# nico-bohlinger/RL-X

Hardware: AMD Instinct MI355X
Metric: env-steps/sec (whole node) PPO 4096 envs at 1/2/4/8 MI355X (higher is better)
Workload: dtype f32

## Files before the change

### rl-x_amd/csrc/gemm_bx.hip

```cpp
#include "gemm_bx.h"
#ifndef RLX_WS_MIN_WAVES
#define RLX_WS_MIN_WAVES 2
#endif
#include "mlp.h"

namespace rlx {

__global__ __launch_bounds__(256) void k_bx_wfrag(BxJobs jobs) {
  int ji = 0;
#pragma unroll
  for (int q = 1; q < BX_MAX_JOBS; ++q)
    if (q < jobs.n && (int)blockIdx.x >= jobs.job[q].first_block) ji = q;
  const BxJob& jb = jobs.job[ji];
  const int idx = ((int)blockIdx.x - jb.first_block) * 256 + threadIdx.x;
  if (idx >= jb.KB * jb.NT * 64) return;
  const int lane = idx & 63, blk = idx >> 6, nt = blk % jb.NT, kb = blk / jb.NT;
  const int j = nt * 32 + (lane & 31), k0 = kb * 16 + 8 * (lane >> 5);
  float v[8];
#pragma unroll
  for (int e = 0; e < 8; ++e) {
    const int k = k0 + e;
    v[e] = (k < jb.K && j < jb.N) ? (jb.trans ? jb.W[(int64_t)j * jb.ldw + k] : jb.W[(int64_t)k * jb.ldw + j]) : 0.f;
  }
  u32x4 pl[X_NP];
// ... 128 lines not shown
#pragma unroll
        for (int j = 0; j < 2; ++j)
#pragma unroll
          for (int r = 0; r < 16; ++r) h[j][r] = hsb[(i * 32 + (r & 3) + 8 * (r >> 2)) * ldc + j * 32];
#pragma unroll
        for (int j = 0; j < 2; ++j)
#pragma unroll
          for (int r = 0; r < 16; ++r)
            cb[(i * 32 + (r & 3) + 8 * (r >> 2)) * ldc + j * 32] = acc[i][j][r] * so * act_grad_t<ACT>(h[j][r]);
      }
    } else {
#pragma unroll
      for (int i = 0; i < MI; ++i)
#pragma unroll
        for (int j = 0; j < 2; ++j)
#pragma unroll
          for (int r = 0; r < 16; ++r) cb[(i * 32 + (r & 3) + 8 * (r >> 2)) * ldc + j * 32] = acc[i][j][r] * so;
    }
    return;
  }
#pragma unroll
  for (int j = 0; j < 2; ++j) {
    const int col = n0 + acc_col(wn, j, lane);
    if (col >= N) continue;
#pragma unroll
    for (int i = 0; i < MI; ++i)
#pragma unroll
      for (int r = 0; r < 16; ++r) {
        const int64_t row = m0 + wm * 32 * MI + i * 32 + (r & 3) + 8 * (r >> 2) + 4 * (lane >> 5);
        if (row < M) {
          const int64_t o = row * ldc + col;
          float v = acc[i][j][r] * so;
          if (MODE == 0) v = act_fwd_t<ACT>(v + bv[j]);
          else if (APPLY) v *= act_grad_t<ACT>((Hsrc ? Hsrc : C)[o]);
          C[o] = v;
        }
      }
  }
}

constexpr int XW_THREADS = 512;
struct DwArgs {
  const float* Hp;
  const float* dZ;
  float* partW;
  float* partB;
  const float *Hp1, *dZ1;
  float *partW1, *partB1;
  int64_t M, Mc;
  int Kd, ldh, N, ntk, ntn;
  BxDwRecompute rc;
};
template <bool TWIN, bool REC = false>
__global__ __launch_bounds__(XW_THREADS, 2) void k_gemm_dw_bx(DwArgs a, DwArgs b, int nb0, float sg, float so) {
  extern __shared__ __attribute__((aligned(16))) char lds[];
  int bid = blockIdx.x, nblk = nb0;
  if (bid >= nb0) {
    a = b;
    bid -= nb0;
    nblk = gridDim.x - nb0;
  }
  const float* __restrict__ Hp = a.Hp;
  const float* __restrict__ dZ = a.dZ;
  float* __restrict__ partW = a.partW;
  float* __restrict__ partB = a.partB;
  if (TWIN && blockIdx.y) {
    Hp = a.Hp1;
    dZ = a.dZ1;
    partW = a.partW1;
    partB = a.partB1;
  }
  const int64_t M = a.M, Mc = a.Mc;
  const int Kd = a.Kd, ldh = a.ldh, N = a.N, ntk = a.ntk, ntn = a.ntn;
  const int ntiles = ntk * ntn;
  const int lb = xcd_remap(bid, nblk);
  const int s = lb / ntiles, tile = lb % ntiles;
  const int k0d = (tile / ntn) * G_BM;
  const int n0 = (tile % ntn) * G_BN;
  const int64_t mbeg = (int64_t)s * Mc;
  int64_t mend = mbeg + Mc;
  if (mend > M) mend = M;
  const int t = threadIdx.x, lane = t & 63, wv = t >> 6;
  const int nk = (int)((mend - mbeg + X_BK - 1) / X_BK);
  const bool interior = k0d + G_BM <= Kd && n0 + G_BN <= N;
  float colsum[4] = {0.f, 0.f, 0.f, 0.f};
  const int pt = t & 255, op = pt >> 7, tt = pt & 127, cg = tt & 31, mg = tt >> 5;
  const bool rec = REC && a.rc.X != nullptr;
  if (REC && wv >= 4 && rec && op == 0) {
    const BxDwRecompute& R = a.rc;
    const int wh = wv - 4, li = lane & 31, lh = lane >> 5;
    const int O = R.O;
    const int64_t pdelta = (TWIN && blockIdx.y) ? R.pdelta1 : 0;
    const float* __restrict__ stats = (TWIN && blockIdx.y) ? R.stats1 : R.stats;
    const u32x4* __restrict__ W1x = reinterpret_cast<const u32x4*>((TWIN && blockIdx.y) ? R.W1x1 : R.W1x);
    const float xs = R.xmax ? x_scale_from_max(*R.xmax, X_ASCALE) : X_ASCALE;
    const float xinv = 1.0f / xs;
    u32x4 w1f[2][2][X_NP];
    float bias[2], gam[2], bet[2];
#pragma unroll
    for (int j = 0; j < 2; ++j) {
      const int ctg = (k0d >> 5) + 2 * wh + j;
#pragma unroll
      for (int kb = 0; kb < 2; ++kb)
#pragma unroll
        for (int p = 0; p < X_NP; ++p) w1f[kb][j][p] = W1x[((int64_t)(kb * R.NT1 + ctg) * X_NP + p) * 64 + lane];
      const int col = k0d + 32 * (2 * wh + j) + li;
      bias[j] = R.b1[pdelta + col];
      gam[j] = R.g[pdelta + col];
      bet[j] = R.be[pdelta + col];
    }
    char* xa = lds + 4 * X_OPER + wh * (X_NP * 2048 + 256);
    float* st_l = reinterpret_cast<float*>(xa + X_NP * 2048);
    for (int i = lane; i < X_NP * 2048 / 16; i += 64) reinterpret_cast<u32x4*>(xa)[i] = u32x4{0u, 0u, 0u, 0u};
    constexpr int XC = 9;
    int xr_[XC], xk_[XC];
#pragma unroll
    for (int c = 0; c < XC; ++c) {
      const int e = lane + 64 * c;
      xr_[c] = e / O;
      xk_[c] = e - xr_[c] * O;
    }
    float xv[XC], smean = 0.f, srstd = 0.f;
    auto xload = [&](int kt) {
      const int64_t m0 = mbeg + (int64_t)kt * X_BK;
      const float* xb = R.X + m0 * O;
      const int nvalid = (int)((mend - m0 < X_BK ? mend - m0 : X_BK)) * O;
#pragma unroll
      for (int c = 0; c < XC; ++c) {
        const int e = lane + 64 * c;
        xv[c] = e < nvalid ? xb[e] : 0.f;
      }
      const bool rv = lane < 32 && m0 + lane < mend;
      smean = rv ? stats[m0 + lane] : 0.f;
      srstd = rv ? stats[M + m0 + lane] : 0.f;
    };
    auto produce = [&](int buf) {
#pragma unroll
      for (int c = 0; c < XC; ++c) {
        if (lane + 64 * c < 32 * O) {
          uint32_t p0, p1;
          bx_split2(xv[c] * xs, 0.f, p0, p1);
          char* da = xa + bx_off(xr_[c], xk_[c] >> 3) + (xk_[c] & 7) * 2;
          *reinterpret_cast<uint16_t*>(da) = (uint16_t)p0;
          *reinterpret_cast<uint16_t*>(da + 2048) = (uint16_t)p1;
        }
      }
      if (lane < 32) { st_l[lane] = smean; st_l[32 + lane] = srstd; }
      f32x16 z[2];
#pragma unroll
      for (int j = 0; j < 2; ++j)
#pragma unroll
        for (int r = 0; r < 16; ++r) z[j][r] = bias[j] * (xs * X_WSCALE);
      const int nks = O > 16 ? 2 : 1;
      for (int kb = 0; kb < nks; ++kb) {
        u32x4 xf[X_NP];
#pragma unroll
        for (int p = 0; p < X_NP; ++p) xf[p] = *reinterpret_cast<const u32x4*>(xa + p * 2048 + bx_off(li, 2 * kb + lh));
#pragma unroll
        for (int j = 0; j < 2; ++j) {
          z[j] = __builtin_amdgcn_mfma_f32_32x32x16_f16(__builtin_bit_cast(f16x8, xf[0]), __builtin_bit_cast(f16x8, w1f[kb][j][1]), z[j], 0, 0, 0);
          z[j] = __builtin_amdgcn_mfma_f32_32x32x16_f16(__builtin_bit_cast(f16x8, xf[1]), __builtin_bit_cast(f16x8, w1f[kb][j][0]), z[j], 0, 0, 0);
          z[j] = __builtin_amdgcn_mfma_f32_32x32x16_f16(__builtin_bit_cast(f16x8, xf[0]), __builtin_bit_cast(f16x8, w1f[kb][j][0]), z[j], 0, 0, 0);
        }
      }
      const float zs = xinv * X_WINV;
      char* dst = lds + buf * 2 * X_OPER;
#pragma unroll
      for (int s8 = 0; s8 < 2; ++s8) {
        float4 mv[2], rv[2];
#pragma unroll
        for (int h2 = 0; h2 < 2; ++h2) {
          mv[h2] = *reinterpret_cast<const float4*>(st_l + 16 * s8 + 8 * h2 + 4 * lh);
          rv[h2] = *reinterpret_cast<const float4*>(st_l + 32 + 16 * s8 + 8 * h2 + 4 * lh);
        }
#pragma unroll
        for (int j = 0; j < 2; ++j) {
          float v[8];
#pragma unroll
          for (int e = 0; e < 8; ++e) {
            const float mean = e < 4 ? (&mv[0].x)[e & 3] : (&mv[1].x)[e & 3];
            const float rs = e < 4 ? (&rv[0].x)[e & 3] : (&rv[1].x)[e & 3];
            const float y = fmaf((z[j][8 * s8 + e] * zs - mean) * rs, gam[j], bet[j]);
            v[e] = y > 0.f ? y : __expf(fminf(y, 0.f)) - 1.0f;
          }
          bx_stage_k8<true>(dst, 32 * (2 * wh + j) + li, 2 * s8 + lh, v, X_ASCALE);
        }
      }
    };
    xload(0);
    produce(0);
    if (nk > 1) xload(1);
    __syncthreads();
    for (int kt = 0; kt < nk; ++kt) {
      if (kt + 1 < nk) {
        produce((kt + 1) & 1);
        if (kt + 2 < nk) xload(kt + 2);
      }
      __syncthreads();
    }
    if (k0d == 0 && partB) {
      const float* red = reinterpret_cast<const float*>(lds);
      __syncthreads();
      if (pt < 128 && n0 + pt < N) partB[(int64_t)s * N + n0 + pt] = (red[pt] + red[128 + pt]) + (red[256 + pt] + red[384 + pt]);
    }
    return;
  }
  if (wv >= 4) {
    const float* __restrict__ src = op ? dZ : Hp;
    const int ld = op ? N : ldh, c0 = (op ? n0 : k0d) + cg * 4, ncols = op ? N : Kd;
    const bool plain = interior && (mend - mbeg) % X_BK == 0;
    float4 rra[8];
    const int rbase = rec ? 16 * (mg >> 1) + 4 * (mg & 1) : mg * 8;
    const float* sp = src + (mbeg + rbase) * ld + c0;
    auto load_plain = [&](int kt, float4 (&rr)[8]) {
      const int64_t m0 = (int64_t)kt * X_BK;
#pragma unroll
      for (int e = 0; e < 8; ++e) rr[e] = *reinterpret_cast<const float4*>(sp + (m0 + (rec ? (e & 3) + 8 * (e >> 2) : e)) * ld);
    };
    auto load_edge = [&](int kt, float4 (&rr)[8]) {
      const int64_t m0 = (int64_t)kt * X_BK;
#pragma unroll
      for (int e = 0; e < 8; ++e) rr[e] = ld4(src, mbeg + m0 + rbase + (rec ? (e & 3) + 8 * (e >> 2) : e), c0, mend, ncols, ld);
    };
    const float sc = op ? sg : X_ASCALE;
    auto stage = [&](int buf, const float4 (&rr)[8]) {
      char* dst = lds + buf * 2 * X_OPER + op * X_OPER;
      float v[8];
#pragma unroll
      for (int e = 0; e < 8; ++e) v[e] = rr[e].x;
      bx_stage_k8<true>(dst, cg * 4 + 0, mg, v, sc);
      if (op) {
#pragma unroll
        for (int e = 0; e < 8; ++e) colsum[0] += v[e];
      }
#pragma unroll
      for (int e = 0; e < 8; ++e) v[e] = rr[e].y;
      bx_stage_k8<true>(dst, cg * 4 + 1, mg, v, sc);
      if (op) {
#pragma unroll
        for (int e = 0; e < 8; ++e) colsum[1] += v[e];
      }
#pragma unroll
      for (int e = 0; e < 8; ++e) v[e] = rr[e].z;
      bx_stage_k8<true>(dst, cg * 4 + 2, mg, v, sc);
      if (op) {
#pragma unroll
        for (int e = 0; e < 8; ++e) colsum[2] += v[e];
      }
#pragma unroll
      for (int e = 0; e < 8; ++e) v[e] = rr[e].w;
      bx_stage_k8<true>(dst, cg * 4 + 3, mg, v, sc);
      if (op) {
// ... 383 lines not shown
    RLX_HIP_TRY(hipFuncSetAttribute(reinterpret_cast<const void*>(k_gemm_dw_bx<true>), hipFuncAttributeMaxDynamicSharedMemorySize,
                                    4 * X_OPER + 16384));
    RLX_HIP_TRY(hipFuncSetAttribute(reinterpret_cast<const void*>(k_gemm_dw_bx<false, true>), hipFuncAttributeMaxDynamicSharedMemorySize,
                                    4 * X_OPER + 16384));
    RLX_HIP_TRY(hipFuncSetAttribute(reinterpret_cast<const void*>(k_gemm_dw_bx<true, true>), hipFuncAttributeMaxDynamicSharedMemorySize,
                                    4 * X_OPER + 16384));
    attr_set.mark();  
  }
  return RLX_OK;
}

static DwArgs dw_args(const float* Hp, const float* dZ, float* pW, float* pB, int64_t M, int Kd, int ldh, int N, int64_t Mc, int ntk,
                      int ntn, const Twin* tw) {
  DwArgs a;
  a.Hp = Hp; a.dZ = dZ; a.partW = pW; a.partB = pB;
  a.Hp1 = tw ? static_cast<const float*>(tw->p[0]) : nullptr;
  a.dZ1 = tw ? static_cast<const float*>(tw->p[1]) : nullptr;
  a.partW1 = tw ? const_cast<float*>(static_cast<const float*>(tw->p[2])) : nullptr;
  a.partB1 = tw ? const_cast<float*>(static_cast<const float*>(tw->p[3])) : nullptr;
  a.M = M; a.Mc = Mc; a.Kd = Kd; a.ldh = ldh; a.N = N; a.ntk = ntk; a.ntn = ntn;
  a.rc = BxDwRecompute{};
  return a;
}
constexpr size_t DW_REC_LDS = 2 * (X_NP * 2048 + 256);

int bx_launch_dw(rlx_ctx* ctx, const float* Hp, const float* dZ, float* pW, float* pB, int64_t M, int Kd, int ldh, int N,
                 int64_t Mc, int S, int ntk, int ntn, hipStream_t st, const Twin* tw) {
  int rc = dw_attr();
  if (rc) return rc;
  const float gs = ctx->bx_gscale;
  ProfScope prof(ctx, PK_GEMM_DW, (tw ? 4.0 : 2.0) * (double)M * Kd * N, st, (tw ? 2.0 : 1.0) * gemm_bytes(Kd, N, M), Kd, N, (int)M, 1);
  const DwArgs a = dw_args(Hp, dZ, pW, pB, M, Kd, ldh, N, Mc, ntk, ntn, tw);
  const int nb = S * ntk * ntn;
  if (tw) {
    RLX_PLAUNCH(k_gemm_dw_bx<true>, dim3(nb, 2), dim3(XW_THREADS), 4 * X_OPER, st, a, a, nb, gs, X_AINV / gs);
  } else {
    RLX_PLAUNCH(k_gemm_dw_bx<false>, dim3(nb), dim3(XW_THREADS), 4 * X_OPER, st, a, a, nb, gs, X_AINV / gs);
  }
  RLX_LAUNCH_CHECK();
  return RLX_OK;
}

int bx_launch_dw2(rlx_ctx* ctx, const BxDwJob& j0, const BxDwJob& j1, int64_t M, hipStream_t st, const Twin* tw0, const Twin* tw1) {
  int rc = dw_attr();
  if (rc) return rc;
  RLX_REQUIRE((tw0 == nullptr) == (tw1 == nullptr), RLX_EINVAL, "bx_launch_dw2: both jobs or neither must have a twin");
  const float gs = ctx->bx_gscale;
  const double nets = tw0 ? 2.0 : 1.0;
  ProfScope prof(ctx, PK_GEMM_DW, nets * 2.0 * (double)M * ((double)j0.Kd * j0.N + (double)j1.Kd * j1.N), st,
                 nets * (gemm_bytes(j0.Kd, j0.N, M) + gemm_bytes(j1.Kd, j1.N, M)), j0.Kd + j1.Kd, j0.N + j1.N, (int)M, 1);
  DwArgs a = dw_args(j0.Hp, j0.dZ, j0.pW, j0.pB, M, j0.Kd, j0.ldh, j0.N, j0.Mc, j0.ntk, j0.ntn, tw0);
  const DwArgs b = dw_args(j1.Hp, j1.dZ, j1.pW, j1.pB, M, j1.Kd, j1.ldh, j1.N, j1.Mc, j1.ntk, j1.ntn, tw1);
  if (j0.rc) {
    RLX_REQUIRE(j0.rc->X && j0.rc->W1x && j0.rc->stats && j0.Kd == 512 && j0.rc->O <= 32 && (!tw0 || (j0.rc->W1x1 && j0.rc->stats1)),
                RLX_EINVAL, "bx_launch_dw2: incomplete recompute description");
    a.rc = *j0.rc;
  }
  const int nb0 = j0.S * j0.ntk * j0.ntn, nb1 = j1.S * j1.ntk * j1.ntn;
  const size_t lds = 4 * X_OPER + (j0.rc ? DW_REC_LDS : 0);
  if (j0.rc) {
    if (tw0) { RLX_PLAUNCH((k_gemm_dw_bx<true, true>), dim3(nb0 + nb1, 2), dim3(XW_THREADS), lds, st, a, b, nb0, gs, X_AINV / gs); }
    else { RLX_PLAUNCH((k_gemm_dw_bx<false, true>), dim3(nb0 + nb1), dim3(XW_THREADS), lds, st, a, b, nb0, gs, X_AINV / gs); }
  } else if (tw0) {
    RLX_PLAUNCH(k_gemm_dw_bx<true>, dim3(nb0 + nb1, 2), dim3(XW_THREADS), lds, st, a, b, nb0, gs, X_AINV / gs);
  } else {
    RLX_PLAUNCH(k_gemm_dw_bx<false>, dim3(nb0 + nb1), dim3(XW_THREADS), lds, st, a, b, nb0, gs, X_AINV / gs);
  }
  RLX_LAUNCH_CHECK();
  return RLX_OK;
}

}
```

### rl-x_amd/csrc/mlp.h

```cpp
#pragma once
#include "gemm.h"

namespace rlx {

constexpr int REDUCE_MAX_SEGS = 48;
constexpr int REDUCE_MAX_BLOCKS = 4096;

struct ReduceSeg {
  const float* src;
  float* dst;
  int64_t len;
  int64_t stride;
  int S;
  int nblocks;
  float scale;
  float bias;
  int in_norm;
  int vec;
};
struct ReduceTable {
  int n;
  ReduceSeg seg[REDUCE_MAX_SEGS];
};

// ... 82 lines not shown
int launch_fwd3h(rlx_ctx* ctx, const rlx_mlp_desc& d, const MlpLayout& L, const float* params, const void* const* wx, const float* x, int ldx,
                 float* z1, float* h1, float* h2, float* h3, float* out, int64_t M, hipStream_t st, const Fwd3hTwin* tw = nullptr);
struct Dxa2hTwin {
  const float* params;
  const void* w2t;
  const float *h1, *h2, *dq;
  float* da;
};
bool dxa2h_supported(const rlx_ctx* ctx, const rlx_mlp_desc& d, int64_t M, int nc);
int launch_dxa2h(rlx_ctx* ctx, const rlx_mlp_desc& d, const MlpLayout& L, const float* params, const void* w2t, const float* h1,
                 const float* h2, const float* dq, float* da, int c0, int nc, int ld_da, int64_t M, hipStream_t st,
                 const Dxa2hTwin* tw = nullptr);
bool dw_merge_ok(const rlx_ctx* ctx, const rlx_mlp_desc& d, const MlpLayout& L, int64_t M);
size_t l1fused_partial_floats(const rlx_mlp_desc& d, int grid);
int l1fused_grid(int64_t M, int num_cus);
struct L1FusedTwin {
  const float* params;
  const float* dZ2;
  float* arena;
  float* grads;
  const void *w2x, *w1x;
  ReduceTable* tab;
};
bool l1fused_bx_images(const rlx_ctx* ctx, const MlpLayout& L, const float* params, const void** w2x, const void** w1x);
int launch_l1fused(rlx_ctx* ctx, const rlx_mlp_desc& d, const MlpLayout& L, const float* params, const float* x,
                   const float* dZ2, float* arena, int grid, float* grads, int64_t M, ReduceTable* tab, hipStream_t st,
                   const L1FusedTwin* tw = nullptr);

int bx_prepare_mlp(rlx_ctx* ctx, const rlx_mlp_desc& d, const MlpLayout& L, const float* params, bool with_bwd, hipStream_t st);
void bx_release(rlx_ctx* ctx);
struct BxNetSpec {
  const rlx_mlp_desc* d;
  const float* params;
  bool with_bwd;
  bool first_layer;
};
int bx_prepare_nets(rlx_ctx* ctx, const BxNetSpec* nets, int n_nets, hipStream_t st, ScratchSlot slot = SL_WFRAG, bool launch = true);
struct BxMat {
  const float* W;
  int K, N;
  bool fwd, trans;
};
int bx_prepare_mats(rlx_ctx* ctx, const BxMat* mats, int n, hipStream_t st);
void bx_release_all(rlx_ctx* ctx);
const void* bx_lookup(const rlx_ctx* ctx, const float* W, int trans, int K, int N);
bool bx_twin_usable(const rlx_ctx* ctx, int64_t M, int N);
int bx_launch_fwd(rlx_ctx* ctx, const float* A, const void* img, const float* bias, float* C, int64_t M, int N, int K, int act,
                  hipStream_t st, int lda, const int32_t* m_dev, const Twin* tw = nullptr);
int bx_launch_dx(rlx_ctx* ctx, const float* dZ, const void* img, float* HD, int64_t M, int N, int Kd, int ldo, int act, int apply,
                 hipStream_t st, const Twin* tw = nullptr, const float* hsrc = nullptr);
bool bx_dw_usable(const rlx_ctx* ctx, int64_t M, int Kd, int ldh, int N);
int bx_launch_dw(rlx_ctx* ctx, const float* Hp, const float* dZ, float* pW, float* pB, int64_t M, int Kd, int ldh, int N,
                 int64_t Mc, int S, int ntk, int ntn, hipStream_t st, const Twin* tw = nullptr);
struct BxDwRecompute {
  const float* X = nullptr;
  const void* W1x = nullptr;
  const float* b1 = nullptr;
  const float* g = nullptr;
  const float* be = nullptr;
  const float* stats = nullptr;
  const uint32_t* xmax = nullptr;
  const void* W1x1 = nullptr;
  const float* stats1 = nullptr;
  int64_t pdelta1 = 0;
  int O = 0, NT1 = 16;
};
struct BxDwJob {
  const float* Hp;
  const float* dZ;
  float *pW, *pB;
  int Kd, ldh, N;
  int64_t Mc;
  int S, ntk, ntn;
  const BxDwRecompute* rc = nullptr;
};
int bx_launch_dw2(rlx_ctx* ctx, const BxDwJob& j0, const BxDwJob& j1, int64_t M, hipStream_t st, const Twin* tw0 = nullptr,
                  const Twin* tw1 = nullptr);


struct BxEmitLayer {
  int64_t w_off;
  int in, out;
  void* nn;
  void* tt;
  int nt_nn, nt_tt;
};
struct BxEmit {
  int n;
  BxEmitLayer l[3];
};
BxEmit bx_emit_table(const rlx_ctx* ctx, const rlx_mlp_desc& d, const float* params);
int launch_clip_adam(float* params, const float* grads, float* m, float* v, int64_t n, const float* sumsq_partials,
                     int n_partials, int64_t step, float lr, float max_norm, float b1, float b2, float eps,
                     float* norm_out, hipStream_t st, const float* sched_dev = nullptr, const BxEmit* emit = nullptr,
                     float* polyak_target = nullptr, float tau = 0.f,
                     float weight_decay = 0.f,
                     int clip_mode = 0);
int launch_clip_adam2(float* p0, const float* g0, float* m0, float* v0, int64_t n0, const float* part0, int np0, float* norm0,
                      const BxEmit* e0, float* p1, const float* g1, float* m1, float* v1, int64_t n1, const float* part1, int np1,
                      float* norm1, const BxEmit* e1, int64_t step, float lr, float max_norm, float b1, float b2, float eps,
                      hipStream_t st, const float* sched_dev = nullptr);
int launch_sumsq_partials2(const float* g0, int64_t n0, float* part0, int* np0, const float* g1, int64_t n1, float* part1, int* np1,
                           hipStream_t st);
int clip_adam_step(rlx_ctx* ctx, float* params, const float* grads, float* m, float* v, int64_t n_params, int64_t step, float lr,
                   float max_grad_norm, float b1, float b2, float eps, float* grad_norm_out, hipStream_t st, const BxEmit* emit);
void adam_schedule_entry(float* out3, int64_t step, float lr, float b1, float b2);
// ... 4 lines not shown
```

### rl-x_amd/csrc/ppo.hip

```cpp
#include "ppo_internal.h"
#include "gemm_bx.h"
#include "dist.h"

namespace rlx {

constexpr float LOG_2PI = 1.8378770664093453f;
constexpr float HALF_LOG_2PIE = 1.4189385332046727f;
constexpr int HEAD_ROWS = 64;

__global__ __launch_bounds__(256) void k_gather(const float* __restrict__ states, const float* __restrict__ actions,
                                                const float* __restrict__ logp, const float* __restrict__ returns,
                                                const float* __restrict__ adv, const int32_t* __restrict__ idx,
                                                float* __restrict__ mb_x, float* __restrict__ mb_a,
                                                float* __restrict__ aux, const int32_t* __restrict__ valid_rows,
                                                int64_t mb, int O, int A, const float* __restrict__ cstates,
                                                float* __restrict__ mb_xc, int Oc) {
  const int64_t nv = valid_rows ? (int64_t)*valid_rows : mb;
  const int64_t nx = mb * O, na = mb * A, nxc = cstates ? mb * Oc : 0;
  const int64_t total = nx + na + mb + nxc;
  for (int64_t e = (int64_t)blockIdx.x * 256 + threadIdx.x; e < total; e += (int64_t)gridDim.x * 256) {
    if (e >= nx + na + mb) {
      const int64_t f = e - nx - na - mb;
      const int64_t r = f / Oc;
      const int d = (int)(f - r * Oc);
// ... 1153 lines not shown
    if (REFILL) {                                                                                                     \
      _Pragma("unroll") for (int j = 0; j < JW; ++j) _Pragma("unroll") for (int p = 0; p < X_NP; ++p)                  \
          bc[u][j][p] = wt[(int64_t)((QU) + PFC) * wstep + (j * X_NP + p) * 64];                                       \
    }                                                                                                                 \
    __builtin_amdgcn_sched_barrier(0);                                                                                \
  }
    static_assert(NBC % PFC == 0 && NBC >= PFC, "phase C: whole groups of PFC blocks");
#pragma unroll 1
    for (int q = 0; q < NBC - PFC; q += PFC) {
#pragma unroll
      for (int u = 0; u < PFC; ++u) T32C_BLOCK(q + u, true)
    }
#pragma unroll
    for (int u = 0; u < PFC; ++u) T32C_BLOCK(NBC - PFC + u, false)
#undef T32C_BLOCK
    const float so2 = X_WINV / gs;
#pragma unroll
    for (int j = 0; j < JW; ++j) {
      const int col = (w * JW + j) * 32 + li;
      float* cb = n.dZ2 + (m0 + 4 * lh) * N2 + col;
      const char* hb = H2P + (4 * lh) * HROW + col * 2;
#pragma unroll
      for (int rr = 0; rr < 16; ++rr) {
        const int rho = (rr & 3) + 8 * (rr >> 2);
        const _Float16 hi = *reinterpret_cast<const _Float16*>(hb + rho * HROW);
        const _Float16 lo = *reinterpret_cast<const _Float16*>(hb + rho * HROW + HPL);
        const float h2 = ((float)hi + (float)lo) * X_AINV;
        cb[(int64_t)rho * N2] = acc[j][rr] * so2 * act_grad_t<ACT>(h2);
      }
    }
  }
}

template <int ACT, int N2>
__global__ __launch_bounds__(256, 2) void k_tail32_bx(TailNet p, TailNet c, const float* __restrict__ mb_a,
                                                      const float* __restrict__ aux, const double* __restrict__ stats,
                                                      float* __restrict__ metrics, int64_t M, float inv_mb, float clip,
                                                      float ent_coef, float critic_coef, const int32_t* __restrict__ valid_rows,
                                                      float gs, int both, int which) {
  extern __shared__ __attribute__((aligned(16))) char tl32_smem[];
  const bool critic = both ? blockIdx.y != 0 : which != 0;
  if (!critic)
    tail32_body<true, ACT, N2>(p, tl32_smem, mb_a, aux, stats, metrics, M, inv_mb, clip, ent_coef, critic_coef, valid_rows, gs);
  else
    tail32_body<false, ACT, N2>(c, tl32_smem, mb_a, aux, stats, metrics, M, inv_mb, clip, ent_coef, critic_coef, valid_rows, gs);
}

static inline int tail_rows(const rlx_ctx* ctx, int N2, int act, int64_t mb) {
  const bool can32 = N2 == 256 && act == RLX_ACT_ELU && mb % T32_ROWS == 0;
  const bool want32 = ctx->ppo_tail == 2 || (ctx->ppo_tail < 0 && (mb <= 8192 || mb > 16384));
  return (can32 && want32) ? T32_ROWS : HEAD_ROWS;
}

static bool tail_shape_ok(const rlx_ctx* ctx, const rlx_mlp_desc& d, int64_t mb, const rlx_ppo_hparams& hp) {
  return ctx->ppo_tail && ctx->gemm_bx && !hp.discrete_actions && d.n_hidden == 3 && d.hidden[2] == TL_K3 && d.hidden[1] % G_BN == 0 &&
         d.hidden[1] <= 512 && d.out_dim <= 8 && mb >= 4096 && mb % HEAD_ROWS == 0;
}

static int launch_tail(rlx_ctx* ctx, const TailNet* p, const TailNet* c, const MbScratch& s, float* metrics, int64_t mb, int N2,
                       int mb_global, const rlx_ppo_hparams& hp, int act, hipStream_t st) {
  const TailNet dummy{};
  const TailNet& tp = p ? *p : dummy;
  const TailNet& tc = c ? *c : dummy;
  const int both = (p && c) ? 1 : 0, which = p ? 0 : 1;
  const float gs = bx_grad_scale(mb_global);
  const float inv_mb = 1.0f / (float)mb_global;
  const size_t lds = 2 * X_OPER + (size_t)HEAD_ROWS * TL_TS * sizeof(float);
  const double nets = both ? 2.0 : 1.0;
  ProfScope prof(s.valid_rows ? nullptr : ctx, PK_TAIL, nets * 4.0 * (double)mb * N2 * TL_K3, st,
                 nets * 4.0 * ((double)mb * (2 * N2 + TL_K3) + 2.0 * N2 * TL_K3), mb, TL_K3, N2, 1);
  if (tail_rows(ctx, N2, act, mb) == T32_ROWS) {
    constexpr int HPL = T32_ROWS * (2 * 256 + 16), DPL = T32_ROWS * (2 * TL_K3 + 16);
    constexpr int TREG = (T32_ROWS * TL_TS * 4 > 2 * DPL) ? T32_ROWS * TL_TS * 4 : 2 * DPL;
    const size_t lds32 = 2 * HPL + TREG + ((size_t)TL_K3 * 8 + 2 * T32_ROWS * 8 + 16 + 2 * TL_K3 * 8) * sizeof(float);
    static AttrOnce attr32;
    if (!attr32.done()) {
      RLX_HIP_TRY(hipFuncSetAttribute(reinterpret_cast<const void*>(k_tail32_bx<RLX_ACT_ELU, 256>),
                                      hipFuncAttributeMaxDynamicSharedMemorySize, 160 * 1024));
      attr32.mark();
    }
    RLX_PLAUNCH((k_tail32_bx<RLX_ACT_ELU, 256>), dim3((unsigned)(mb / T32_ROWS), both ? 2 : 1), dim3(256), lds32, st, tp, tc, s.mb_a,
                s.aux, s.stats, metrics, mb, inv_mb, hp.clip_range, hp.entropy_coef, hp.critic_coef, s.valid_rows, gs, both, which);
    RLX_LAUNCH_CHECK();
    return RLX_OK;
  }
#define RLX_TAIL_LAUNCH(ACTV)                                                                                        \
  {                                                                                                                  \
    static AttrOnce attr_set;                                                                                          \
    if (!attr_set.done()) {                                                                                                 \
      RLX_HIP_TRY(hipFuncSetAttribute(reinterpret_cast<const void*>(k_tail_bx<ACTV>),                                \
                                      hipFuncAttributeMaxDynamicSharedMemorySize, 160 * 1024));                      \
      attr_set.mark();                                                                                                 \
    }                                                                                                                \
    RLX_PLAUNCH((k_tail_bx<ACTV>), dim3((unsigned)(mb / HEAD_ROWS), both ? 2 : 1), dim3(256), lds, st, tp, tc, s.mb_a, s.aux,   \
                s.stats, metrics, mb, N2, inv_mb, hp.clip_range, hp.entropy_coef, hp.critic_coef, s.valid_rows, gs, both,      \
                which);                                                                                              \
  }
  if (act == RLX_ACT_ELU) RLX_TAIL_LAUNCH(RLX_ACT_ELU)
  else if (act == RLX_ACT_TANH) RLX_TAIL_LAUNCH(RLX_ACT_TANH)
  else RLX_TAIL_LAUNCH(RLX_ACT_RELU)
#undef RLX_TAIL_LAUNCH
  RLX_LAUNCH_CHECK();
  return RLX_OK;
}

template <bool POLICY>
// ... 23 lines not shown
      RLX_HIP_TRY(hipFuncSetAttribute(reinterpret_cast<const void*>(k_head_loss_fast<POLICY, KQV>),              \
                                      hipFuncAttributeMaxDynamicSharedMemorySize, 160 * 1024));                 \
      attr_set.mark();                                                                                            \
    }                                                                                                           \
    RLX_PLAUNCH((k_head_loss_fast<POLICY, KQV>), dim3(nb), dim3(256), lds, st, H, W, b, logstd, s.mb_a, s.aux,          \
                s.stats, s.head_part, metrics, mb, A, PS, inv_mb, hp.clip_range, hp.entropy_coef, hp.critic_coef,        \
                act, s.valid_rows);                                                                             \
  }
    if (K == 64) RLX_HL_FAST(16)
    else if (K == 128) RLX_HL_FAST(32)
    else RLX_HL_FAST(64)
#undef RLX_HL_FAST
    RLX_LAUNCH_CHECK();
    return RLX_OK;
  }
  const size_t lds = ((size_t)HEAD_ROWS * (K + 1) + (size_t)K * A + 2 * (size_t)HEAD_ROWS * A + 2 * A) * sizeof(float);
  RLX_REQUIRE(lds <= 160 * 1024, RLX_EUNSUP, "ppo head: last hidden layer too wide for the LDS-staged head kernel");
  hipLaunchKernelGGL(k_head_loss<POLICY>, dim3(nb), dim3(256), lds, st, H, W, b, logstd, s.mb_a, s.aux, s.stats, s.head_part,
                     metrics, mb, K, A, PS, inv_mb, hp.clip_range, hp.entropy_coef, hp.critic_coef, act, s.valid_rows);
  RLX_LAUNCH_CHECK();
  return RLX_OK;
}

template <bool POLICY>
static int net_fwd_bwd(rlx_ctx* ctx, const rlx_mlp_desc& d, const float* params, float* grads, float* metrics,
                       const MbScratch& s, int64_t mb, int mb_global, const rlx_ppo_hparams& hp, float* sumsq,
                       int* n_sumsq, hipStream_t st, hipEvent_t ev_after_fwd = nullptr) {
  const MlpLayout L = make_layout(d);
  const bool kept = ctx->bx_keep[ctx->bank] && ctx->bx_n[ctx->bank] > 0 && d.n_hidden >= 2 &&
                    ctx->bx_img[ctx->bank][0].W == params + L.layer[1].W;
  int rc = (mb >= 4096 && !kept) ? bx_prepare_mlp(ctx, d, L, params, true, st) : RLX_OK;
  if (rc) return rc;
  struct BxScope { rlx_ctx* c; ~BxScope() { if (!c->bx_keep[c->bank]) bx_release(c); } } bx_scope{ctx};
  const float* x_in = (!POLICY && s.mb_xc) ? s.mb_xc : s.mb_x;
  const int K = L.head.in, A = L.head.out;
  const int PS = K * A + 2 * A + 8;
  int nb = div_up(mb, HEAD_ROWS);
  const float inv_mb = 1.0f / (float)mb_global;
  const bool discrete = POLICY && hp.discrete_actions != 0;
  const void *w3f = nullptr, *w3t = nullptr;
  float* dz2 = nullptr;
  if (tail_shape_ok(ctx, d, mb, hp)) {
    const LayerOff& o3 = L.layer[2];
    w3f = bx_lookup(ctx, params + o3.W, 0, o3.in, o3.out);
    w3t = bx_lookup(ctx, params + o3.W, 1, o3.out, o3.in);
    if (w3f && w3t) dz2 = (float*)scratch(ctx, SL_DACT_0, (size_t)mb * o3.in * sizeof(float));
  }
  const bool tail = dz2 != nullptr;
  if (tail) nb = (int)(mb / tail_rows(ctx, L.layer[2].in, d.act, mb));
  XmaxScope xscope(ctx, ctx->xmax_slot[(!POLICY && s.mb_xc) ? 1 : 0]);
  struct L12Scope { rlx_ctx* c; ~L12Scope() { c->l12_stats = nullptr; c->l12_ran = false; } } l12scope{ctx};
  ctx->l12_ran = false;
  ctx->l12_stats = nullptr;
  if (ctx->dw_recompute && tail && ctx->l12_fused && l12fwd_supported(d) && dw_merge_ok(ctx, d, L, mb) && d.hidden[0] == 512 &&
      d.act == RLX_ACT_ELU && grads) {
    ctx->l12_stats = (float*)scratch(ctx, SL_LN_P, (size_t)2 * mb * sizeof(float));
    if (!ctx->l12_stats) return RLX_ENOMEM;
  }
  rc = mlp_trunk_fwd(ctx, d, L, params, x_in, s.acts, mb, st, 0, false, nullptr, tail ? d.n_hidden - 1 : -1);
  if (rc) return rc;
  if (ev_after_fwd) RLX_HIP_TRY(hipEventRecord(ev_after_fwd, st));
  if (tail) {
    const LayerOff& o3 = L.layer[2];
    const TailNet tn{s.acts[1], (const u32x4*)w3f, (const u32x4*)w3t, params + o3.b, params + L.head.W, params + L.head.b,
                     POLICY ? params + L.logstd : nullptr, s.acts[2], dz2, s.head_part, A, PS};
    rc = launch_tail(ctx, POLICY ? &tn : nullptr, POLICY ? nullptr : &tn, s, metrics, mb, o3.in, mb_global, hp, d.act, st);
  } else {
    rc = launch_head_loss<POLICY>(s.acts[d.n_hidden - 1], params + L.head.W, params + L.head.b,
                                  (POLICY && !discrete) ? params + L.logstd : nullptr, s, metrics, mb, K, A, PS, inv_mb, hp,
                                  d.act, st, ctx);
  }
  if (rc) return rc;
  ReduceSeg extra[8];
  int ne = 0;
  extra[ne++] = ReduceSeg{s.head_part, grads + L.head.W, (int64_t)K * A, (int64_t)PS, nb, 0, 1.f, 0.f, 1};
  extra[ne++] = ReduceSeg{s.head_part + K * A, grads + L.head.b, (int64_t)A, (int64_t)PS, nb, 0, 1.f, 0.f, 1};
  if (POLICY) {
    if (!discrete)
      extra[ne++] = ReduceSeg{s.head_part + K * A + A, grads + L.logstd, (int64_t)A, (int64_t)PS, nb, 0, 1.f, 0.f, 1};
    else
      extra[ne++] = ReduceSeg{s.head_part + K * A + 2 * A + 3, metrics + 2, 1, (int64_t)PS, nb, 0, inv_mb, 0.f, 0};
    extra[ne++] = ReduceSeg{s.head_part + K * A + 2 * A + 0, metrics + 0, 1, (int64_t)PS, nb, 0, inv_mb, 0.f, 0};
    extra[ne++] = ReduceSeg{s.head_part + K * A + 2 * A + 1, metrics + 3, 1, (int64_t)PS, nb, 0, inv_mb, 0.f, 0};
    extra[ne++] = ReduceSeg{s.head_part + K * A + 2 * A + 2, metrics + 4, 1, (int64_t)PS, nb, 0, inv_mb, 0.f, 0};
  } else {
    extra[ne++] = ReduceSeg{s.head_part + K * A + 2 * A + 0, metrics + 1, 1, (int64_t)PS, nb, 0, inv_mb, 0.f, 0};
  }
  GradScaleScope gscope(ctx, bx_grad_scale(mb_global));
  TrunkOpts topt;
  topt.dz_below_last = dz2;
  return mlp_trunk_bwd(ctx, d, L, params, x_in, s.acts, grads, mb, extra, ne, sumsq, n_sumsq, st, tail ? &topt : nullptr);
}

struct XmaxCall {
  rlx_ctx* c;
  explicit XmaxCall(rlx_ctx* ctx) : c(ctx) {}
  int set(const float* states, int64_t n, const float* cstates, int64_t nc, hipStream_t st) {
    if (!c->gemm_bx) return RLX_OK;
    int rc = x_max_update(c, states, n, 0, st, &c->xmax_slot[0]);
    if (!rc && cstates) rc = x_max_update(c, cstates, nc, 1, st, &c->xmax_slot[1]);
    return rc;
  }
  ~XmaxCall() { c->xmax_slot[0] = c->xmax_slot[1] = nullptr; }
};

static bool twin_shapes_ok(const rlx_ctx* ctx, const rlx_mlp_desc& pd, const rlx_mlp_desc& cd, const rlx_ppo_hparams& hp,
                           int64_t mb) {
  if (ctx->ppo_twin == 0 || (ctx->ppo_twin < 0 && mb > 16384)) return false;
// ... 12 lines not shown
  if (!(K == 64 || K == 128 || K == 256)) return false;
  if (mb < 4096 || !l1fwd_mfma_supported(pd) || !l1fused_supported(pd)) return false;
  for (int l = 1; l < pd.n_hidden; ++l)
    if (!bx_dw_usable(ctx, mb, pd.hidden[l - 1], pd.hidden[l - 1], pd.hidden[l])) return false;
  return true;
}

struct TwinImages {
  const void* f[4][2];
  const void* t[4][2];
  const void* w2x[2];
  const void* w1x[2];
};

static int twin_images(rlx_ctx* ctx, const rlx_mlp_desc& pd, const MlpLayout& LP, const float* pparams, const rlx_mlp_desc& cd,
                       const MlpLayout& LC, const float* cparams, hipStream_t st, TwinImages* im, bool* ok) {
  *ok = false;
  const rlx_mlp_desc* dd[2] = {&pd, &cd};
  const MlpLayout* LL[2] = {&LP, &LC};
  const float* pp[2] = {pparams, cparams};
  const int bank0 = ctx->bank;
  for (int q = 0; q < 2; ++q) {
    ctx->bank = q;
    const bool kept = ctx->bx_keep[q] && ctx->bx_n[q] > 0 && ctx->bx_img[q][0].W == pp[q] + LL[q]->layer[1].W;
    if (!kept) {
      const int rc = bx_prepare_mlp(ctx, *dd[q], *LL[q], pp[q], true, st);
      if (rc) { ctx->bank = bank0; return rc; }
    }
    bool all = l1fused_bx_images(ctx, *LL[q], pp[q], &im->w2x[q], &im->w1x[q]);
    for (int l = 1; l < dd[q]->n_hidden && all; ++l) {
      const LayerOff& o = LL[q]->layer[l];
      im->f[l][q] = bx_lookup(ctx, pp[q] + o.W, 0, o.in, o.out);
      im->t[l][q] = bx_lookup(ctx, pp[q] + o.W, 1, o.out, o.in);
      all = im->f[l][q] && im->t[l][q];
    }
    if (!all) { ctx->bank = bank0; return RLX_OK; }
  }
  ctx->bank = bank0;
  *ok = true;
  return RLX_OK;
}

static int twin_fwd_bwd(rlx_ctx* ctx, const rlx_mlp_desc& pd, const MlpLayout& LP, const float* pparams, float* pg,
                        const rlx_mlp_desc& cd, const MlpLayout& LC, const float* cparams, float* cg, const TwinImages& im,
                        float* met, const MbScratch& sp, const MbScratch& sc, int64_t mb, int mb_global,
                        const rlx_ppo_hparams& hp, float* sq, int* npb, int* ncb, hipStream_t st) {
  const int nh = pd.n_hidden, last = nh - 1;
  Twin t;
  XmaxScope xscope(ctx, ctx->xmax_slot[0]);
  int rc;
  int l_first = 1;
  float* stats2[2] = {nullptr, nullptr};
  const bool l12 = ctx->l12_fused && l12fwd_supported(pd) && im.w1x[0] && im.w1x[1];
  if (l12 && ctx->dw_recompute && ctx->dw_merge && nh == 3 && tail_shape_ok(ctx, pd, mb, hp) && pd.hidden[0] == 512 &&
      pd.act == RLX_ACT_ELU) {
    const int b0 = ctx->bank;
    for (int q = 0; q < 2; ++q) {
      ctx->bank = q;
      stats2[q] = (float*)scratch(ctx, SL_LN_P, (size_t)2 * mb * sizeof(float));
    }
    ctx->bank = b0;
    if (!stats2[0] || !stats2[1]) return RLX_ENOMEM;
  }
  if (l12) {
    L12Twin tw{cparams, sc.acts[0], sc.acts[1], im.w1x[1], im.f[1][1]};
    tw.stats = stats2[1];
    rc = launch_l12fwd(ctx, pd, LP, pparams, sp.mb_x, sp.acts[0], sp.acts[1], im.w1x[0], im.f[1][0], mb, st, &tw, stats2[0]);
    l_first = 2;
  } else {
    rc = launch_l1fwd_mfma(pd, LP, pparams, sp.mb_x, sp.acts[0], mb, ctx->num_cus, st, nullptr, ctx, cparams, sc.acts[0]);
  }
  if (rc) return rc;
  float* dz2[2] = {nullptr, nullptr};
  const float* dzb[4][2];
  for (int l = 0; l < 4; ++l) { dzb[l][0] = sp.acts[l]; dzb[l][1] = sc.acts[l]; }
  if (tail_shape_ok(ctx, pd, mb, hp)) {
    const int bank0_ = ctx->bank;
    for (int q = 0; q < 2; ++q) {
      ctx->bank = q;
      dz2[q] = (float*)scratch(ctx, SL_DACT_0, (size_t)mb * LP.layer[2].in * sizeof(float));
    }
    ctx->bank = bank0_;
    if (!dz2[0] || !dz2[1]) return RLX_ENOMEM;
    dzb[1][0] = dz2[0];
    dzb[1][1] = dz2[1];
  }
  const bool tail = dz2[0] != nullptr;
  for (int l = l_first; l < (tail ? nh - 1 : nh); ++l) {
    const LayerOff& o = LP.layer[l];
    t.p[0] = sc.acts[l - 1]; t.p[1] = im.f[l][1]; t.p[2] = cparams + LC.layer[l].b; t.p[3] = sc.acts[l];
    rc = bx_launch_fwd(ctx, sp.acts[l - 1], im.f[l][0], pparams + o.b, sp.acts[l], mb, o.out, o.in, pd.act, st, 0, nullptr, &t);
    if (rc) return rc;
  }
  const int K = LP.head.in, A = LP.head.out;
  const int PSp = K * A + 2 * A + 8, PSc = K + 2 + 8;
  const int nb = tail ? (int)(mb / tail_rows(ctx, LP.layer[2].in, pd.act, mb)) : div_up(mb, HEAD_ROWS);
  const float inv_mb = 1.0f / (float)mb_global;
  if (tail) {
    const LayerOff& o3 = LP.layer[2];
    const TailNet tp{sp.acts[1], (const u32x4*)im.f[2][0], (const u32x4*)im.t[2][0], pparams + o3.b, pparams + LP.head.W,
                     pparams + LP.head.b, pparams + LP.logstd, sp.acts[2], dz2[0], sp.head_part, A, PSp};
    const TailNet tc{sc.acts[1], (const u32x4*)im.f[2][1], (const u32x4*)im.t[2][1], cparams + LC.layer[2].b, cparams + LC.head.W,
                     cparams + LC.head.b, nullptr, sc.acts[2], dz2[1], sc.head_part, 1, PSc};
    rc = launch_tail(ctx, &tp, &tc, sp, met, mb, o3.in, mb_global, hp, pd.act, st);
    if (rc) return rc;
  } else {
    const HeadNet hn_p{sp.acts[last], pparams + LP.head.W, pparams + LP.head.b, pparams + LP.logstd, sp.head_part, A, PSp};
    const HeadNet hn_c{sc.acts[last], cparams + LC.head.W, cparams + LC.head.b, nullptr, sc.head_part, 1, PSc};
// ... 976 lines not shown
```

Before: 7.692 million.

## Slim recompute producer registers and pipeline X loads in dW GEMM

```diff
diff --git a/rl-x_amd/csrc/gemm_bx.hip b/rl-x_amd/csrc/gemm_bx.hip
--- a/rl-x_amd/csrc/gemm_bx.hip
+++ b/rl-x_amd/csrc/gemm_bx.hip
@@ -204,7 +204,7 @@
   BxDwRecompute rc;
 };
 template <bool TWIN, bool REC = false>
-__global__ __launch_bounds__(XW_THREADS, 2) void k_gemm_dw_bx(DwArgs a, DwArgs b, int nb0, float sg, float so) {
+__global__ __launch_bounds__(XW_THREADS, REC ? 4 : 2) void k_gemm_dw_bx(DwArgs a, DwArgs b, int nb0, float sg, float so) {
   extern __shared__ __attribute__((aligned(16))) char lds[];
   int bid = blockIdx.x, nblk = nb0;
   if (bid >= nb0) {
@@ -243,19 +243,27 @@
     const int wh = wv - 4, li = lane & 31, lh = lane >> 5;
     const int O = R.O;
     const int64_t pdelta = (TWIN && blockIdx.y) ? R.pdelta1 : 0;
-    const float* __restrict__ stats = (TWIN && blockIdx.y) ? R.stats1 : R.stats;
-    const u32x4* __restrict__ W1x = reinterpret_cast<const u32x4*>((TWIN && blockIdx.y) ? R.W1x1 : R.W1x);
+    typedef const float __attribute__((address_space(1)))* gf_t;
+    typedef const u32x4 __attribute__((address_space(1)))* gfrag_t;
+    const gf_t X = (gf_t)R.X;
+    const gf_t stats = (gf_t)((TWIN && blockIdx.y) ? R.stats1 : R.stats);
+    const gfrag_t w1b = (gfrag_t)((TWIN && blockIdx.y) ? R.W1x1 : R.W1x) + ((int64_t)((k0d >> 5) + 2 * wh) * X_NP) * 64 + lane;
     const float xs = R.xmax ? x_scale_from_max(*R.xmax, X_ASCALE) : X_ASCALE;
     const float xinv = 1.0f / xs;
-    u32x4 w1f[2][2][X_NP];
+    u32x4 w1f[2][X_NP];
+    uint32_t w1h[2][X_NP];
+    auto wload = [&]() {
+#pragma unroll
+      for (int j = 0; j < 2; ++j)
+#pragma unroll
+        for (int p = 0; p < X_NP; ++p) {
+          w1f[j][p] = w1b[((int64_t)j * X_NP + p) * 64];
+          w1h[j][p] = *reinterpret_cast<const uint32_t __attribute__((address_space(1)))*>(w1b + ((int64_t)(R.NT1 + j) * X_NP + p) * 64);
+        }
+    };
     float bias[2], gam[2], bet[2];
 #pragma unroll
     for (int j = 0; j < 2; ++j) {
-      const int ctg = (k0d >> 5) + 2 * wh + j;
-#pragma unroll
-      for (int kb = 0; kb < 2; ++kb)
-#pragma unroll
-        for (int p = 0; p < X_NP; ++p) w1f[kb][j][p] = W1x[((int64_t)(kb * R.NT1 + ctg) * X_NP + p) * 64 + lane];
       const int col = k0d + 32 * (2 * wh + j) + li;
       bias[j] = R.b1[pdelta + col];
       gam[j] = R.g[pdelta + col];
@@ -264,55 +272,58 @@
     char* xa = lds + 4 * X_OPER + wh * (X_NP * 2048 + 256);
     float* st_l = reinterpret_cast<float*>(xa + X_NP * 2048);
     for (int i = lane; i < X_NP * 2048 / 16; i += 64) reinterpret_cast<u32x4*>(xa)[i] = u32x4{0u, 0u, 0u, 0u};
-    constexpr int XC = 9;
-    int xr_[XC], xk_[XC];
-#pragma unroll
-    for (int c = 0; c < XC; ++c) {
-      const int e = lane + 64 * c;
-      xr_[c] = e / O;
-      xk_[c] = e - xr_[c] * O;
-    }
-    float xv[XC], smean = 0.f, srstd = 0.f;
+    constexpr int XC = (BX_DW_REC_MAX_O + 1) / 2;
+    float xv[XC], smean, srstd;
+    typedef const char __attribute__((address_space(1)))* gb_t;
     auto xload = [&](int kt) {
-      const int64_t m0 = mbeg + (int64_t)kt * X_BK;
-      const float* xb = R.X + m0 * O;
-      const int nvalid = (int)((mend - m0 < X_BK ? mend - m0 : X_BK)) * O;
-#pragma unroll
-      for (int c = 0; c < XC; ++c) {
-        const int e = lane + 64 * c;
-        xv[c] = e < nvalid ? xb[e] : 0.f;
-      }
-      const bool rv = lane < 32 && m0 + lane < mend;
-      smean = rv ? stats[m0 + lane] : 0.f;
-      srstd = rv ? stats[M + m0 + lane] : 0.f;
-    };
-    auto produce = [&](int buf) {
-#pragma unroll
-      for (int c = 0; c < XC; ++c) {
-        if (lane + 64 * c < 32 * O) {
-          uint32_t p0, p1;
-          bx_split2(xv[c] * xs, 0.f, p0, p1);
-          char* da = xa + bx_off(xr_[c], xk_[c] >> 3) + (xk_[c] & 7) * 2;
-          *reinterpret_cast<uint16_t*>(da) = (uint16_t)p0;
-          *reinterpret_cast<uint16_t*>(da + 2048) = (uint16_t)p1;
+      const int64_t m0 = mbeg + (int64_t)(kt < nk ? kt : nk - 1) * X_BK;
+      const int nrows = (int)(mend - m0 < X_BK ? mend - m0 : X_BK);
+      const uint32_t r = (uint32_t)(li < nrows ? li : nrows - 1), ro = r * (uint32_t)O * 4u, last = ((uint32_t)(nrows * O) - 1u) * 4u;
+      const gb_t xb = (gb_t)(X + m0 * O);
+#pragma unroll
+      for (int i = 0; i < XC; ++i) {
+        const uint32_t o = ro + 4u * (uint32_t)(lh + 2 * i);
+        xv[i] = *(gf_t)(xb + (o < last ? o : last));
+      }
+      const gb_t sb = (gb_t)(stats + m0);
+      smean = *(gf_t)(sb + 4u * r);
+      srstd = *(gf_t)(sb + (int64_t)M * 4 + 4u * r);
+    };
+    auto produce = [&](int buf, int kt_next) {
+      char* xrow = xa + li * X_ROWB + 2 * lh;
+      const int sw = (li >> 2) & 3;
+#pragma unroll
+      for (int i = 0; i < XC; ++i) {
+        uint32_t p0, p1;
+        bx_split2(lh + 2 * i < O ? xv[i] * xs : 0.f, 0.f, p0, p1);
+        char* da = xrow + ((((i >> 2) ^ sw)) << 4) + 4 * (i & 3);
+        *reinterpret_cast<uint16_t*>(da) = (uint16_t)p0;
+        *reinterpret_cast<uint16_t*>(da + 2048) = (uint16_t)p1;
+      }
+      st_l[li] = smean;
+      st_l[32 + li] = srstd;
+      xload(kt_next);
+      __builtin_amdgcn_sched_barrier(0);
+      f32x16 z[2];
+#pragma unroll
+      for (int j = 0; j < 2; ++j)
+#pragma unroll
+        for (int r = 0; r < 16; ++r) z[j][r] = bias[j] * (xs * X_WSCALE);
+#pragma unroll
+      for (int kb = 0; kb < 2; ++kb) {
+        if (kb == 1 && O <= 16) break;
+        u32x4 xf[X_NP], wf[2][X_NP];
+#pragma unroll
+        for (int p = 0; p < X_NP; ++p) {
+          xf[p] = *reinterpret_cast<const u32x4*>(xa + p * 2048 + bx_off(li, 2 * kb + lh));
+#pragma unroll
+          for (int j = 0; j < 2; ++j) wf[j][p] = kb == 0 ? w1f[j][p] : u32x4{lh ? 0u : w1h[j][p], 0u, 0u, 0u};
         }
-      }
-      if (lane < 32) { st_l[lane] = smean; st_l[32 + lane] = srstd; }
-      f32x16 z[2];
-#pragma unroll
-      for (int j = 0; j < 2; ++j)
-#pragma unroll
-        for (int r = 0; r < 16; ++r) z[j][r] = bias[j] * (xs * X_WSCALE);
-      const int nks = O > 16 ? 2 : 1;
-      for (int kb = 0; kb < nks; ++kb) {
-        u32x4 xf[X_NP];
-#pragma unroll
-        for (int p = 0; p < X_NP; ++p) xf[p] = *reinterpret_cast<const u32x4*>(xa + p * 2048 + bx_off(li, 2 * kb + lh));
 #pragma unroll
         for (int j = 0; j < 2; ++j) {
-          z[j] = __builtin_amdgcn_mfma_f32_32x32x16_f16(__builtin_bit_cast(f16x8, xf[0]), __builtin_bit_cast(f16x8, w1f[kb][j][1]), z[j], 0, 0, 0);
-          z[j] = __builtin_amdgcn_mfma_f32_32x32x16_f16(__builtin_bit_cast(f16x8, xf[1]), __builtin_bit_cast(f16x8, w1f[kb][j][0]), z[j], 0, 0, 0);
-          z[j] = __builtin_amdgcn_mfma_f32_32x32x16_f16(__builtin_bit_cast(f16x8, xf[0]), __builtin_bit_cast(f16x8, w1f[kb][j][0]), z[j], 0, 0, 0);
+          z[j] = __builtin_amdgcn_mfma_f32_32x32x16_f16(__builtin_bit_cast(f16x8, xf[0]), __builtin_bit_cast(f16x8, wf[j][1]), z[j], 0, 0, 0);
+          z[j] = __builtin_amdgcn_mfma_f32_32x32x16_f16(__builtin_bit_cast(f16x8, xf[1]), __builtin_bit_cast(f16x8, wf[j][0]), z[j], 0, 0, 0);
+          z[j] = __builtin_amdgcn_mfma_f32_32x32x16_f16(__builtin_bit_cast(f16x8, xf[0]), __builtin_bit_cast(f16x8, wf[j][0]), z[j], 0, 0, 0);
         }
       }
       const float zs = xinv * X_WINV;
@@ -338,18 +349,17 @@
           bx_stage_k8<true>(dst, 32 * (2 * wh + j) + li, 2 * s8 + lh, v, X_ASCALE);
         }
       }
+      wload();
     };
     xload(0);
-    produce(0);
-    if (nk > 1) xload(1);
+    wload();
+    produce(0, 1);
     __syncthreads();
-    for (int kt = 0; kt < nk; ++kt) {
-      if (kt + 1 < nk) {
-        produce((kt + 1) & 1);
-        if (kt + 2 < nk) xload(kt + 2);
-      }
+    for (int kt = 0; kt + 1 < nk; ++kt) {
+      produce((kt + 1) & 1, kt + 2);
       __syncthreads();
     }
+    __syncthreads();
     if (k0d == 0 && partB) {
       const float* red = reinterpret_cast<const float*>(lds);
       __syncthreads();
@@ -839,7 +849,7 @@
   DwArgs a = dw_args(j0.Hp, j0.dZ, j0.pW, j0.pB, M, j0.Kd, j0.ldh, j0.N, j0.Mc, j0.ntk, j0.ntn, tw0);
   const DwArgs b = dw_args(j1.Hp, j1.dZ, j1.pW, j1.pB, M, j1.Kd, j1.ldh, j1.N, j1.Mc, j1.ntk, j1.ntn, tw1);
   if (j0.rc) {
-    RLX_REQUIRE(j0.rc->X && j0.rc->W1x && j0.rc->stats && j0.Kd == 512 && j0.rc->O <= 32 && (!tw0 || (j0.rc->W1x1 && j0.rc->stats1)),
+    RLX_REQUIRE(j0.rc->X && j0.rc->W1x && j0.rc->stats && j0.Kd == 512 && j0.rc->O <= BX_DW_REC_MAX_O && (!tw0 || (j0.rc->W1x1 && j0.rc->stats1)),
                 RLX_EINVAL, "bx_launch_dw2: incomplete recompute description");
     a.rc = *j0.rc;
   }
diff --git a/rl-x_amd/csrc/mlp.h b/rl-x_amd/csrc/mlp.h
--- a/rl-x_amd/csrc/mlp.h
+++ b/rl-x_amd/csrc/mlp.h
@@ -158,6 +158,7 @@
 bool bx_dw_usable(const rlx_ctx* ctx, int64_t M, int Kd, int ldh, int N);
 int bx_launch_dw(rlx_ctx* ctx, const float* Hp, const float* dZ, float* pW, float* pB, int64_t M, int Kd, int ldh, int N,
                  int64_t Mc, int S, int ntk, int ntn, hipStream_t st, const Twin* tw = nullptr);
+constexpr int BX_DW_REC_MAX_O = 18;
 struct BxDwRecompute {
   const float* X = nullptr;
   const void* W1x = nullptr;
diff --git a/rl-x_amd/csrc/ppo.hip b/rl-x_amd/csrc/ppo.hip
--- a/rl-x_amd/csrc/ppo.hip
+++ b/rl-x_amd/csrc/ppo.hip
@@ -1229,6 +1229,10 @@
   return (can32 && want32) ? T32_ROWS : HEAD_ROWS;
 }
 
+static bool dw_recompute_on(const rlx_ctx* ctx, const rlx_mlp_desc& d) {
+  return ctx->dw_recompute && d.in_dim <= BX_DW_REC_MAX_O && d.hidden[0] == 512 && d.act == RLX_ACT_ELU;
+}
+
 static bool tail_shape_ok(const rlx_ctx* ctx, const rlx_mlp_desc& d, int64_t mb, const rlx_ppo_hparams& hp) {
   return ctx->ppo_tail && ctx->gemm_bx && !hp.discrete_actions && d.n_hidden == 3 && d.hidden[2] == TL_K3 && d.hidden[1] % G_BN == 0 &&
          d.hidden[1] <= 512 && d.out_dim <= 8 && mb >= 4096 && mb % HEAD_ROWS == 0;
@@ -1358,8 +1362,7 @@
   struct L12Scope { rlx_ctx* c; ~L12Scope() { c->l12_stats = nullptr; c->l12_ran = false; } } l12scope{ctx};
   ctx->l12_ran = false;
   ctx->l12_stats = nullptr;
-  if (ctx->dw_recompute && tail && ctx->l12_fused && l12fwd_supported(d) && dw_merge_ok(ctx, d, L, mb) && d.hidden[0] == 512 &&
-      d.act == RLX_ACT_ELU && grads) {
+  if (dw_recompute_on(ctx, d) && tail && ctx->l12_fused && l12fwd_supported(d) && dw_merge_ok(ctx, d, L, mb) && grads) {
     ctx->l12_stats = (float*)scratch(ctx, SL_LN_P, (size_t)2 * mb * sizeof(float));
     if (!ctx->l12_stats) return RLX_ENOMEM;
   }
@@ -1478,8 +1481,7 @@
   int l_first = 1;
   float* stats2[2] = {nullptr, nullptr};
   const bool l12 = ctx->l12_fused && l12fwd_supported(pd) && im.w1x[0] && im.w1x[1];
-  if (l12 && ctx->dw_recompute && ctx->dw_merge && nh == 3 && tail_shape_ok(ctx, pd, mb, hp) && pd.hidden[0] == 512 &&
-      pd.act == RLX_ACT_ELU) {
+  if (l12 && dw_recompute_on(ctx, pd) && ctx->dw_merge && nh == 3 && tail_shape_ok(ctx, pd, mb, hp)) {
     const int b0 = ctx->bank;
     for (int q = 0; q < 2; ++q) {
       ctx->bank = q;
```

Result: no change. 7.665 million, median of 2 (-0.4%).
